# clearmatics/libff

Hardware: AMD Instinct MI355X
Metric: G1 MSM throughput (scalar-muls/sec) (higher is better)
Workload: dtype u32

## Files before the change

libff_amd/csrc/engine.cpp:

```cpp
#include "../../include/amdmsm.h"
#include "engine_internal.h"
#include "group_vtable.h"

#include <hip/hip_runtime.h>

#include <fcntl.h>
#include <sys/stat.h>
#include <unistd.h>

#include <algorithm>
#include <cmath>
#include <cstdio>
#include <cstdlib>
#include <cstring>
#include <mutex>
#include <string>
#include <thread>
#include <vector>

using namespace amdmsm;

constexpr int MAX_SLOTS = 4;
constexpr int MAX_GROUPS = 4;
struct ws_slot {
// ... 207 lines not shown
    while (L < 64u && (size_t)p.W * (size_t)batch * p.B * red_lanes / L > (size_t)70000) L <<= 1;
    if (L_req > 0) L = (uint32_t)L_req;
    while (L > p.B) L >>= 1;
    if (L == 0 || (L & (L - 1))) return AMDMSM_ERR_BAD_ARG;
    p.L = L;
    const size_t xyz_bytes = (size_t)3 * vt->el_words * 4;
    p.list_stride = align_up(n ? n : 1, 64) + 16;
    {
        const double resident = (double)vt->accumulate_resident_lanes(overlap ? 1 : 0);
        const double entries = (double)n * p.W;
        uint32_t S = 8;
        if (entries >= 4.0 * 256.0 * resident) {
            S = 256;
        } else if (entries >= 8.0 * 128.0 * resident) {
            S = 128;
        } else if (entries > 8.0 * resident) {
            uint32_t k = 1;
            while (entries / (k * resident) > 128.0) ++k;
            S = (uint32_t)std::ceil(entries / (k * resident));
            while (S < 128 && (double)p.W * (double)((n + S - 1) / S) > k * resident) ++S;
        }
        if (S_req > 0) S = (uint32_t)S_req;
        p.S = S;
        p.T = (uint32_t)((n + S - 1) / S);
        if (p.T == 0) p.T = 1;
    }
    p.K = batch;
    const size_t Wt = (size_t)p.W * (size_t)batch;
    size_t off = 0;
    p.off_counts = off;
    off = align_up(off + Wt * p.B * 4, 256);
    p.off_lists = off;
    off = align_up(off + Wt * p.list_stride * 4, 256);
    const size_t zz_bytes = (size_t)vt->bucket_words * 4;
    p.off_buckets = off;
    off = align_up(off + Wt * p.B * zz_bytes, 256);
    const size_t M = p.B / p.L;
    p.off_lvl0 = off;
    off = align_up(off + Wt * M * xyz_bytes, 256);
    p.off_lvl1 = off;
    off = align_up(off + Wt * (M / 2 + 1) * xyz_bytes, 256);
    p.off_pfirst = off;
    off = align_up(off + Wt * p.T * zz_bytes, 256);
    p.off_plast = off;
    off = align_up(off + Wt * p.T * zz_bytes, 256);
    p.off_cont = off;
    off = align_up(off + Wt * p.T * 4, 256);
    p.G = G_req > 0 ? std::min(std::min(G_req, MAX_GROUPS), p.W) : 1;
    p.off_queue = off;
    p.queue_stride = align_up(fixup_queue_words((size_t)((p.W + p.G - 1) / p.G) * (size_t)batch * p.T) * 4, 256);
    off = off + p.queue_stride * p.G;
    p.off_partial = off;
    off = align_up(off + (size_t)MAX_GROUPS * xyz_bytes, 256);
    p.off_coarse = off;
    off = align_up(off + Wt * 1025 * 4, 256);
    p.off_big = off;
    p.big_stride = p.c <= 22 ? align_up(sort_geometry(n, p.c, p.W).big_words * 4, 256) : 256;
    off += p.big_stride * (size_t)batch;
    p.off_cursor = off;
    off = align_up(off + Wt * 1024 * 4, 256);
    p.off_tmp_payload = off;
    off = align_up(off + Wt * p.list_stride * 4, 256);
    p.off_tmp_key = off;
    off = align_up(off + Wt * p.list_stride * 4, 256);
    p.off_endo = off;
    p.endo_stride = glv ? align_up((n / 2) * (size_t)vt->el_words * 2 * 4, 256) : 0;
    off += p.endo_stride * (size_t)batch;
    {
        static const int rc_env = getenv("AMDMSM_ROWCOL") ? atoi(getenv("AMDMSM_ROWCOL")) : 1;
        static const int rc_min_c = getenv("AMDMSM_ROWCOL_MIN_C") ? atoi(getenv("AMDMSM_ROWCOL_MIN_C")) : 10;
        static const int qr_env = getenv("AMDMSM_ROWCOL_QROW") ? atoi(getenv("AMDMSM_ROWCOL_QROW")) : 0;
        static const int qc_env = getenv("AMDMSM_ROWCOL_QCOL") ? atoi(getenv("AMDMSM_ROWCOL_QCOL")) : 0;
        p.rowcol = rc_env != 0 && p.c >= rc_min_c;
        const int h = p.c / 2;
        const size_t C = (size_t)1 << h, R = p.B >> h;
        const bool one_wave = vt->fq_words >= 24 || vt->el_words > vt->fq_words;
        const size_t lane_budget = one_wave ? 70000 : 140000;
        uint32_t q = 4;
        while (q < 64 && Wt * p.B * red_lanes * 2 / q > lane_budget) q <<= 1;
        p.q_row = qr_env > 0 ? (uint32_t)qr_env : q;
        p.q_col = qc_env > 0 ? (uint32_t)qc_env : q;
        p.rc_points = R + 1 + C;
        p.off_rc = off;
        off = align_up(off + Wt * p.rc_points * xyz_bytes, 256);
        p.off_planes = off;
        off = align_up(off + Wt * p.c * xyz_bytes, 256);
        p.off_winsum = off;
        off = align_up(off + Wt * xyz_bytes, 256);
    }
    p.total = off;
    return AMDMSM_OK;
}

int ensure_ws(amdmsm_ctx *ctx, ws_slot &sl, size_t bytes) {
    if (sl.ws_bytes >= bytes) return AMDMSM_OK;
    if (sl.ws) {
        HIP_TRY(ctx, hipDeviceSynchronize());
        HIP_TRY(ctx, hipFree(sl.ws));
        sl.ws = nullptr;
        sl.ws_bytes = 0;
    }
    const size_t want = bytes + bytes / 8;
    HIP_TRY(ctx, hipMalloc(&sl.ws, want));
    sl.ws_bytes = want;
    return AMDMSM_OK;
}

constexpr uint64_t TIMING_RING = 64;
void record(amdmsm_ctx *ctx, ws_slot &sl, int idx, hipStream_t st) {
    (void)sl;
    if (ctx->timing) (void)hipEventRecord(ctx->ring[ctx->ticket % TIMING_RING][idx], st);
}

bool use_endomorphism(const group_vtable *vt, size_t n, const amdmsm_opts *opts, int table_digits) {
    static const int env = [] {
        const char *e = getenv("AMDMSM_GLV");
        int v = 0;
        if (!e) return 0;
        if (!strcmp(e, "off") || !strcmp(e, "0")) v = -1;
        else if (!strcmp(e, "on") || !strcmp(e, "1")) v = 1;
        else if (!strcmp(e, "all") || !strcmp(e, "force") || !strcmp(e, "2")) v = 2;
        else if (!strcmp(e, "auto")) v = 3;
        if (v) fprintf(stderr, "[amdmsm] AMDMSM_GLV=%s overrides amdmsm_opts.endomorphism where the caller left it at 0 "
                               "(off: everywhere); on / force assert that every base lies in the order-r subgroup\n", e);
        return v;
    }();
    if (!vt->has_endomorphism) return false;
    if (table_digits || n == 0 || n >= ((size_t)1 << 30)) return false;
    const int c_req = opts ? opts->window_bits : 0;
    if (c_req > 22) return false;
    int want = opts ? opts->endomorphism : 0;
    if (env == -1) want = -1;
    else if ((env == 1 || env == 2) && want == 0) want = env;
    if (want < 0 || (want == 0 && !vt->prime_order)) return false;
    if (want >= 2) return true;
    double full = 0, split = 0;
    if (c_req) {
        full = plan_cost(vt, n, c_req, false);
        split = plan_cost(vt, n, c_req, true);
    } else {
        choose_c(vt, n, false, &full);
        choose_c(vt, n, true, &split);
    }
    return split < 0.98 * full;
}

int check_opts(amdmsm_ctx *ctx, const amdmsm_opts *opts) {
    if (opts && opts->struct_size != sizeof(amdmsm_opts))
        return fail(ctx, AMDMSM_ERR_BAD_ARG, "amdmsm_opts.struct_size does not match this library (AMDMSM_ABI_VERSION " +
                                                 std::to_string(AMDMSM_ABI_VERSION) + "): initialise with AMDMSM_OPTS_INIT");
    return AMDMSM_OK;
}
#define CHECK_OPTS(ctx, opts)                       \
    do {                                            \
        const int rc_opts_ = check_opts(ctx, opts); \
        if (rc_opts_) return rc_opts_;              \
    } while (0)

constexpr size_t MAX_RANGES = 64;
size_t max_range_points() {
    static const size_t v = [] {
        const char *e = getenv("AMDMSM_MAX_RANGE_POINTS");
        const long long x = e ? atoll(e) : 0;
        return x > 0 ? (size_t)x : (size_t)1 << 28;
    }();
    return v;
}
// ... 27 lines not shown
                       groups_env, glv, overlap);
    if (rc) return fail(ctx, rc, "bad window_bits / segment_len");
    const int slot_idx = (int)(ctx->next++ % (unsigned)ctx->depth);
    ws_slot &sl = ctx->slots[slot_idx];
    ctx->last_slot = slot_idx;
    if (overlap) {
        HIP_TRY(ctx, hipEventRecord(sl.ov_in, user_st));
        st = ctx->bulk_stream;
        HIP_TRY(ctx, hipStreamWaitEvent(st, sl.ov_in, 0));
    }
    if (sl.used) HIP_TRY(ctx, hipStreamWaitEvent(st, sl.done, 0));
    rc = ensure_ws(ctx, sl, p.total);
    if (rc) return rc;
    char *ws = (char *)sl.ws;
    uint32_t *counts = (uint32_t *)(ws + p.off_counts);
    uint32_t *lists = (uint32_t *)(ws + p.off_lists);
    uint32_t *buckets = (uint32_t *)(ws + p.off_buckets);
    uint32_t *lvl0 = (uint32_t *)(ws + p.off_lvl0);
    uint32_t *lvl1 = (uint32_t *)(ws + p.off_lvl1);

    record(ctx, sl, 0, st);
    const uint32_t *endo_pts = !glv ? nullptr : (d_endo_resident ? d_endo_resident : (const uint32_t *)(ws + p.off_endo));
    const bool endo_beside = glv && !d_endo_resident && !(hook && hook->fn);
    HIP_TRY(ctx, hipEventRecord(sl.tail_done[0], st));
    if ((atomic_sort || p.c > 22) && !table_digits) {
        HIP_TRY(ctx, hipMemsetAsync(counts, 0, (size_t)p.W * p.B * 4, st));
        vt->count(st, d_scalars, n, mont, p.c, p.W, counts);
        record(ctx, sl, 1, st);
        vt->scatter(st, d_scalars, n, mont, p.c, p.W, counts, lists, p.list_stride);
    } else {
        HIP_TRY(ctx, hipMemsetAsync(ws + p.off_coarse, 0, p.off_big + 16 - p.off_coarse, st));
        record(ctx, sl, 1, st);
        vt->sort(st, d_scalars, n, mont, p.c, table_digits ? table_digits : p.W, (uint32_t *)(ws + p.off_coarse),
                 (uint32_t *)(ws + p.off_cursor), (int32_t *)lists, (uint32_t *)(ws + p.off_tmp_payload),
                 (uint32_t *)(ws + p.off_tmp_key), counts, lists, p.list_stride, (uint32_t *)(ws + p.off_big),
                 table_digits ? 1 : (glv ? 2 : 0), nullptr);
    }
    hipStream_t side = overlap ? st : sl.side[0];
    if (!overlap) HIP_TRY(ctx, hipStreamWaitEvent(side, sl.tail_done[0], 0));
    HIP_TRY(ctx, hipMemsetAsync(buckets, 0, (size_t)p.W * p.B * vt->bucket_words * 4, side));
    for (int g = 0; g < p.G; ++g) HIP_TRY(ctx, hipMemsetAsync(ws + p.off_queue + g * p.queue_stride, 0, 8, side));
    if (endo_beside) vt->endo_points(side, d_bases, n, (uint32_t *)(ws + p.off_endo));
    if (!overlap) HIP_TRY(ctx, hipEventRecord(sl.acc_done[0], side));
    if (hook && hook->fn) {
        hipEvent_t wait_for = nullptr;
        rc = hook->fn(hook->arg, &wait_for);
        if (rc) return rc;
        if (wait_for) HIP_TRY(ctx, hipStreamWaitEvent(st, wait_for, 0));
    }
    if (!overlap) HIP_TRY(ctx, hipStreamWaitEvent(st, sl.acc_done[0], 0));
    if (glv && !d_endo_resident && !endo_beside) vt->endo_points(st, d_bases, n, (uint32_t *)(ws + p.off_endo));
    const size_t zzw = (size_t)vt->bucket_words, xyzw = (size_t)vt->el_words * 3;
    const size_t M0 = p.B / p.L, cap1 = M0 / 2 + 1;
    uint32_t *pfirst = (uint32_t *)(ws + p.off_pfirst), *plast = (uint32_t *)(ws + p.off_plast);
    uint32_t *cont = (uint32_t *)(ws + p.off_cont), *partial = (uint32_t *)(ws + p.off_partial);
    int w_hi = p.W;
    for (int g = 0; g < p.G; ++g) {
        const int wg = p.W / p.G + (g < p.W % p.G ? 1 : 0);
        const int w0 = w_hi - wg;
        w_hi = w0;
        const bool last = g == p.G - 1;
        hipStream_t ts = last ? (overlap ? ctx->tail_stream : st) : sl.side[g];
        if (g == 0) record(ctx, sl, 2, st);
        vt->accumulate(st, counts + (size_t)w0 * p.B, lists + (size_t)w0 * p.list_stride, p.list_stride, d_bases,
                       buckets + (size_t)w0 * p.B * zzw, pfirst + (size_t)w0 * p.T * zzw, plast + (size_t)w0 * p.T * zzw,
                       cont + (size_t)w0 * p.T, wg, p.B, p.S, p.T, endo_pts, n, overlap ? 1 : 0);
        if (last) {
            record(ctx, sl, 3, st);
            if (overlap) {
                HIP_TRY(ctx, hipEventRecord(sl.ov_acc, st));
                HIP_TRY(ctx, hipStreamWaitEvent(ts, sl.ov_acc, 0));
            }
        } else {
            HIP_TRY(ctx, hipEventRecord(sl.acc_done[g], st));
            HIP_TRY(ctx, hipStreamWaitEvent(ts, sl.acc_done[g], 0));
        }
        vt->accumulate_fixup(ts, counts + (size_t)w0 * p.B, buckets + (size_t)w0 * p.B * zzw,
                             pfirst + (size_t)w0 * p.T * zzw, plast + (size_t)w0 * p.T * zzw, cont + (size_t)w0 * p.T,
                             (uint32_t *)(ws + p.off_queue + g * p.queue_stride), wg, p.B, p.S, p.T);
        uint32_t *src = lvl0 + (size_t)w0 * M0 * xyzw, *dst = lvl1 + (size_t)w0 * cap1 * xyzw;
        if (p.rowcol) {
            src = (uint32_t *)(ws + p.off_winsum) + (size_t)w0 * xyzw;
            vt->reduce_rowcol(ts, buckets + (size_t)w0 * p.B * zzw, wg, p.B, p.c, p.q_row, p.q_col,
                              (uint32_t *)(ws + p.off_rc) + (size_t)w0 * p.rc_points * xyzw,
                              (uint32_t *)(ws + p.off_planes) + (size_t)w0 * p.c * xyzw, src);
        } else {
            vt->reduce_segments(ts, buckets + (size_t)w0 * p.B * zzw, wg, p.B, p.L, src);
            const uint32_t fold = (uint32_t)vt->reduce_fold;
            uint32_t M = (uint32_t)M0;
            M /= std::min<uint32_t>(M, fold);
            while (M > 1) {
                if ((size_t)M * (64 / fold) <= 256) {
                    vt->sum_block(ts, src, wg, M, dst);
                    M = 1;
                } else {
                    vt->sum_butterfly(ts, src, wg, M, dst);
                    M /= std::min<uint32_t>(M, fold);
                }
                std::swap(src, dst);
            }
        }
        if (g > 0) HIP_TRY(ctx, hipStreamWaitEvent(ts, sl.tail_done[g - 1], 0));
        if (last) record(ctx, sl, 4, ts);
        vt->horner(ts, src, wg, p.c, last ? form : (int)AMDMSM_OUT_JACOBIAN, g > 0 ? partial + (size_t)(g - 1) * xyzw : nullptr,
                   last ? d_out : partial + (size_t)g * xyzw);
        if (!last) HIP_TRY(ctx, hipEventRecord(sl.tail_done[g], ts));
    }
    if (overlap) {
        record(ctx, sl, 5, ctx->tail_stream);
        HIP_TRY(ctx, hipEventRecord(sl.ov_tail, ctx->tail_stream));
        HIP_TRY(ctx, hipStreamWaitEvent(user_st, sl.ov_tail, 0));
        st = user_st;
    } else {
        record(ctx, sl, 5, st);
    }
    if (ctx->timing) sl.last_ticket = (long long)ctx->ticket++;
    sl.ev_valid = ctx->timing;
    HIP_TRY(ctx, hipEventRecord(sl.done, st));
    sl.used = true;
    HIP_TRY(ctx, hipGetLastError());
    return AMDMSM_OK;
}

constexpr int MAX_BATCH = 8;
int msm_device_batch_impl(amdmsm_ctx *ctx, const group_vtable *vt, int k, const uint32_t *const *d_bases,
                          const uint32_t *const *d_scalars, size_t n, uint32_t *const *d_outs, const amdmsm_opts *opts) {
    hipStream_t st = (opts && opts->stream) ? (hipStream_t)opts->stream : ctx->stream;
    const int form = opts ? opts->out_form : AMDMSM_OUT_LIBFF;
    const int mont = (opts && opts->scalars_plain) ? 0 : 1;
    const bool glv = use_endomorphism(vt, n, opts, 0);
    const size_t entries = glv ? 2 * n : n;
    plan_t p;
    int rc = make_plan(vt, entries, opts ? opts->window_bits : 0, opts ? opts->segment_len : 0, p, 0, 0, 0, glv, false, k);
    if (rc) return fail(ctx, rc, "bad window_bits / segment_len");
    if (p.c > 22) return fail(ctx, AMDMSM_ERR_BAD_ARG, "window_bits > 22 is not available for a batch");
    const int slot_idx = (int)(ctx->next++ % (unsigned)ctx->depth);
    ws_slot &sl = ctx->slots[slot_idx];
    ctx->last_slot = slot_idx;
    if (sl.used) HIP_TRY(ctx, hipStreamWaitEvent(st, sl.done, 0));
    rc = ensure_ws(ctx, sl, p.total);
    if (rc) return rc;
    char *ws = (char *)sl.ws;
    const size_t zzw = (size_t)vt->bucket_words, xyzw = (size_t)vt->el_words * 3;
    const size_t Wt = (size_t)p.W * (size_t)k;
    uint32_t *counts = (uint32_t *)(ws + p.off_counts), *lists = (uint32_t *)(ws + p.off_lists);
    uint32_t *buckets = (uint32_t *)(ws + p.off_buckets);
    uint32_t *pfirst = (uint32_t *)(ws + p.off_pfirst), *plast = (uint32_t *)(ws + p.off_plast), *cont = (uint32_t *)(ws + p.off_cont);
    record(ctx, sl, 0, st);
    HIP_TRY(ctx, hipMemsetAsync(ws + p.off_coarse, 0, Wt * 1025 * 4, st));
    for (int j = 0; j < k; ++j) HIP_TRY(ctx, hipMemsetAsync(ws + p.off_big + (size_t)j * p.big_stride, 0, 16, st));
    HIP_TRY(ctx, hipMemsetAsync(buckets, 0, Wt * p.B * vt->bucket_words * 4, st));
    HIP_TRY(ctx, hipMemsetAsync(ws + p.off_queue, 0, 8, st));
    record(ctx, sl, 1, st);
    for (int j = 0; j < k; ++j) {
        const size_t w0 = (size_t)j * p.W;
        uint32_t *lists_j = lists + w0 * p.list_stride, *counts_j = counts + w0 * p.B;
        vt->sort(st, d_scalars[j], n, mont, p.c, p.W, (uint32_t *)(ws + p.off_coarse) + w0 * 1025,
                 (uint32_t *)(ws + p.off_cursor) + w0 * 1024, (int32_t *)lists_j,
                 (uint32_t *)(ws + p.off_tmp_payload) + w0 * p.list_stride, (uint32_t *)(ws + p.off_tmp_key) + w0 * p.list_stride,
                 counts_j, lists_j, p.list_stride, (uint32_t *)(ws + p.off_big + (size_t)j * p.big_stride), glv ? 2 : 0, nullptr);
        uint32_t *endo_j = glv ? (uint32_t *)(ws + p.off_endo + (size_t)j * p.endo_stride) : nullptr;
        if (glv) vt->endo_points(st, d_bases[j], n, endo_j);
        if (j == 0) record(ctx, sl, 2, st);
        vt->accumulate(st, counts_j, lists_j, p.list_stride, d_bases[j], buckets + w0 * p.B * zzw, pfirst + w0 * p.T * zzw,
                       plast + w0 * p.T * zzw, cont + w0 * p.T, p.W, p.B, p.S, p.T, endo_j, n, 0);
    }
    record(ctx, sl, 3, st);
// ... 1450 lines not shown
```

libff_amd/csrc/msm_group.hip:

```cpp
#include "curve_params.h"
#include "ec.cuh"
#include "fp2h.cuh"
#include "group_vtable.h"
#include "wide.cuh"
#include "wide28.cuh"
#include "rr.cuh"

#include <algorithm>
#include <cstdio>
#include <vector>
#include <type_traits>

#ifndef AMDMSM_GROUP
#error "compile with -DAMDMSM_GROUP=<group traits> -DAMDMSM_VT=<vtable getter name>"
#endif

namespace amdmsm {
template <bool I>
struct ec_coeff_a<Fp<AMDMSM_GROUP::fq, I>> {
    static constexpr int value = AMDMSM_GROUP::DEG == 1 ? AMDMSM_GROUP::COEFF_A : 0;
};
template <int NR, bool I>
struct ec_coeff_a<Fp2<AMDMSM_GROUP::fq, NR, I>> {
    static constexpr int value = AMDMSM_GROUP::DEG == 2 ? AMDMSM_GROUP::COEFF_A : 0;
// ... 1421 lines not shown
    const uint32_t i = (uint32_t)(t % M);
    const bool valid = w < (size_t)W;
    Jac<ER> p;
    if (valid) load_jac(p, in + t * XYZW); else jac_set_inf(p);
    wave_group_sum_r(p, G);
    if (valid && (i % G) == 0) store_jac(out + (w * (M / G) + i / G) * XYZW, p);
}

__global__ void __launch_bounds__(256) k_sum_block(const uint32_t* __restrict__ in, int W, uint32_t M,
                                                    uint32_t* __restrict__ out) {
    __shared__ uint32_t part[4 * XYZW];
    const size_t w = blockIdx.x;
    const uint32_t i = threadIdx.x / RED_LANES;
    const uint32_t lane = threadIdx.x & 63u, wave = threadIdx.x >> 6, nw = blockDim.x >> 6;
    Jac<ER> p;
    if (i < M) load_jac(p, in + (w * M + i) * XYZW); else jac_set_inf(p);
    wave_group_sum_r(p, RED_FOLD);
    if (lane < (uint32_t)RED_LANES) store_jac(part + wave * XYZW, p);
    __syncthreads();
    if (wave != 0) return;
    const uint32_t j = lane / RED_LANES;
    if (j < nw) load_jac(p, part + j * XYZW); else jac_set_inf(p);
    uint32_t G = 1;
    while (G < nw) G <<= 1;
    wave_group_sum_r(p, G);
    if (lane < (uint32_t)RED_LANES) store_jac(out + w * XYZW, p);
}

constexpr int SUMW_THREADS = (GP::DEG == 1 && FQ::N < 16) ? 512 : 256;
constexpr int SUMW_SLOTS = SUMW_THREADS / RED_LANES / 4;
template <class Q = FQ>
AMDMSM_DEV void sum_wide_add(const WideEnv<Q>& env, const uint32_t* a, const uint32_t* b, uint32_t* o) {
    if constexpr (GP::DEG == 2) {
        using F = WideFq2<Q, (GP::NR_SMALL == 0 ? -1 : GP::NR_SMALL)>;
        const uint32_t wi = F::word_index(env);
        uint32_t X1 = env.valid ? a[wi] : 0u, Y1 = env.valid ? a[EW + wi] : 0u, Z1 = env.valid ? a[2 * EW + wi] : 0u;
        const uint32_t X2 = env.valid ? b[wi] : 0u, Y2 = env.valid ? b[EW + wi] : 0u, Z2 = env.valid ? b[2 * EW + wi] : 0u;
        jac_add_seq<F, Q, GP::COEFF_A>(env, X1, Y1, Z1, X2, Y2, Z2);
        if (((threadIdx.x & 63u) >> 4) < 2 && env.valid) {
            o[wi] = X1;
            o[EW + wi] = Y1;
            o[2 * EW + wi] = Z1;
        }
    } else {
        uint32_t X1 = env.valid ? a[env.j] : 0u, Y1 = env.valid ? a[EW + env.j] : 0u, Z1 = env.valid ? a[2 * EW + env.j] : 0u;
        const uint32_t X2 = env.valid ? b[env.j] : 0u, Y2 = env.valid ? b[EW + env.j] : 0u, Z2 = env.valid ? b[2 * EW + env.j] : 0u;
        if constexpr (Q::N < 16) jac_add_wide<Q, GP::COEFF_A>(env, X1, Y1, Z1, X2, Y2, Z2);
        else jac_add_seq<WideFq<Q>, Q>(env, X1, Y1, Z1, X2, Y2, Z2);
        if ((threadIdx.x & 63u) < (uint32_t)Q::N) {
            o[env.j] = X1;
            o[EW + env.j] = Y1;
            o[2 * EW + env.j] = Z1;
        }
    }
}
__global__ void __launch_bounds__(SUMW_THREADS) k_sum_block_wide(const uint32_t* __restrict__ in, int W, uint32_t M,
                                                                 uint32_t* __restrict__ out) {
    __shared__ uint32_t buf[2][SUMW_SLOTS * XYZW];
    __builtin_amdgcn_s_setprio(3);
    const size_t w = blockIdx.x;
    const uint32_t i = threadIdx.x / RED_LANES, wave = threadIdx.x >> 6;
    constexpr uint32_t NWAVES = SUMW_THREADS / 64;
    Jac<ER> p;
    if (i < M) load_jac(p, in + (w * M + i) * XYZW); else jac_set_inf(p);
    wave_group_sum_r(p, 4);
    if ((i & 3u) == 0) store_jac(buf[0] + (size_t)(i >> 2) * XYZW, p);
    __syncthreads();
    const WideEnv<FQ> env = wide_env<FQ>();
    uint32_t K = (M + 3) / 4;
    int cur = 0;
    while (K > 1) {
        const uint32_t pairs = K / 2;
        for (uint32_t q = wave; q < pairs; q += NWAVES) {
            const uint32_t* a = buf[cur] + (size_t)(2 * q) * XYZW;
            sum_wide_add(env, a, a + XYZW, buf[cur ^ 1] + (size_t)q * XYZW);
        }
        __syncthreads();
        cur ^= 1;
        K = pairs;
    }
    for (uint32_t t = threadIdx.x; t < (uint32_t)XYZW; t += SUMW_THREADS) out[w * XYZW + t] = buf[cur][t];
}

__global__ void __launch_bounds__(64, AMDMSM_TAIL_WAVES) k_bucket_sums(const uint32_t* __restrict__ buckets, int W, uint32_t B, int h,
                                                    uint32_t q_row, uint32_t q_col, uint32_t row_blocks,
                                                    uint32_t* __restrict__ out) {
    __builtin_amdgcn_s_setprio(3);
    const bool col = blockIdx.x >= row_blocks;
    const size_t t = ((size_t)(blockIdx.x - (col ? row_blocks : 0u)) * 64 + threadIdx.x) / RED_LANES;
    const uint32_t C = 1u << h, R = B >> h;
    const uint32_t q = col ? q_col : q_row, len = col ? R : C;
    const uint32_t g = len / q;
    const uint32_t nout = col ? C : R + 1;
    const size_t per_w = (size_t)nout * g;
    const size_t w = t / per_w;
    const uint32_t rem = (uint32_t)(t % per_w), o = rem / g, j = rem % g;
    const bool valid = w < (size_t)W;
    rec_sum sum;
    rec_sum_init(sum);
    if (valid) {
        const uint32_t* bk = buckets + w * (size_t)B * ZZS;
        for (uint32_t i = 0; i < q; ++i) {
            const uint32_t idx = j * q + i;
            const uint64_t b1 = col ? (uint64_t)idx * C + o : (uint64_t)o * C + idx;
            if (b1 >= 1 && b1 <= B) rec_sum_add(sum, bk + (size_t)(b1 - 1) * ZZS);
        }
    }
    rec_sum_fold(sum, g);
    Xyzz<ER> xa;
    rec_sum_get(xa, sum);
    Jac<ER> p;
    xyzz_to_jac(p, xa);
    if (valid && j == 0) store_jac(out + (w * (size_t)(R + 1 + C) + (col ? R + 1 + o : o)) * XYZW, p);
}

__global__ void __launch_bounds__(256) k_plane_sums(const uint32_t* __restrict__ rc, int W, int c, int h,
                                                     uint32_t* __restrict__ planes) {
    __shared__ uint32_t part[4 * XYZW];
    __builtin_amdgcn_s_setprio(3);
    const uint32_t w = blockIdx.x / (uint32_t)c, k = blockIdx.x % (uint32_t)c;
    const uint32_t C = 1u << h, R = (1u << (c - 1)) >> h, NP = R + 1 + C;
    const bool from_cols = k < (uint32_t)h;
    const uint32_t* src = rc + ((size_t)w * NP + (from_cols ? R + 1 : 0)) * XYZW;
    const uint32_t bit = from_cols ? k : k - (uint32_t)h;
    const bool top = k == (uint32_t)c - 1;
    const uint32_t M = top ? 1u : (from_cols ? C : R) / 2;
    const uint32_t nlanes = blockDim.x / RED_LANES, i0 = threadIdx.x / RED_LANES;
    const uint32_t lane = threadIdx.x & 63u, wave = threadIdx.x >> 6, nw = blockDim.x >> 6;
    Jac<ER> p, x;
    jac_set_inf(p);
    for (uint32_t i = i0; i < M; i += nlanes) {
        const uint32_t idx = top ? R : (((i >> bit) << (bit + 1)) | (1u << bit) | (i & ((1u << bit) - 1u)));
        load_jac(x, src + (size_t)idx * XYZW);
        jac_add(p, p, x);
    }
    wave_group_sum_r(p, RED_FOLD);
    if (lane < (uint32_t)RED_LANES) store_jac(part + wave * XYZW, p);
    __syncthreads();
    if (wave != 0) return;
    const uint32_t jw = lane / RED_LANES;
    if (jw < nw) load_jac(p, part + jw * XYZW); else jac_set_inf(p);
    uint32_t G = 1;
    while (G < nw) G <<= 1;
    wave_group_sum_r(p, G);
    if (lane < (uint32_t)RED_LANES) store_jac(planes + ((size_t)w * c + k) * XYZW, p);
}

__global__ void __launch_bounds__(SUMW_THREADS) k_plane_sums_wide(const uint32_t* __restrict__ rc, int W, int c, int h,
                                                                  uint32_t* __restrict__ planes) {
    __shared__ uint32_t buf[2][SUMW_SLOTS * XYZW];
    __builtin_amdgcn_s_setprio(3);
    const uint32_t w = blockIdx.x / (uint32_t)c, k = blockIdx.x % (uint32_t)c;
    const uint32_t C = 1u << h, R = (1u << (c - 1)) >> h, NP = R + 1 + C;
    const bool from_cols = k < (uint32_t)h;
    const uint32_t* src = rc + ((size_t)w * NP + (from_cols ? R + 1 : 0)) * XYZW;
    const uint32_t bit = from_cols ? k : k - (uint32_t)h;
    const bool top = k == (uint32_t)c - 1;
    const uint32_t M = top ? 1u : (from_cols ? C : R) / 2;
    constexpr uint32_t NLANES = SUMW_THREADS / RED_LANES, NWAVES = SUMW_THREADS / 64;
    const uint32_t i0 = threadIdx.x / RED_LANES, wave = threadIdx.x >> 6;
    Jac<ER> p, x;
    jac_set_inf(p);
    for (uint32_t i = i0; i < M; i += NLANES) {
        const uint32_t idx = top ? R : (((i >> bit) << (bit + 1)) | (1u << bit) | (i & ((1u << bit) - 1u)));
        load_jac(x, src + (size_t)idx * XYZW);
        jac_add(p, p, x);
    }
    wave_group_sum_r(p, 4);
    if ((i0 & 3u) == 0) store_jac(buf[0] + (size_t)(i0 >> 2) * XYZW, p);
    __syncthreads();
    const WideEnv<FQ> env = wide_env<FQ>();
    uint32_t K = ((M < NLANES ? M : NLANES) + 3) / 4;
    int cur = 0;
    while (K > 1) {
        const uint32_t pairs = K / 2;
        for (uint32_t q = wave; q < pairs; q += NWAVES) {
            const uint32_t* a = buf[cur] + (size_t)(2 * q) * XYZW;
            sum_wide_add(env, a, a + XYZW, buf[cur ^ 1] + (size_t)q * XYZW);
        }
        __syncthreads();
        cur ^= 1;
        K = pairs;
    }
    for (uint32_t t = threadIdx.x; t < (uint32_t)XYZW; t += SUMW_THREADS) planes[((size_t)w * c + k) * XYZW + t] = buf[cur][t];
}

template <class P, bool I>
AMDMSM_DEV typename std::enable_if<(P::N < 16), void>::type horner_chain(Jac<Fp<P, I>>& res,
                                                                         const uint32_t* __restrict__ window_sums, int W,
                                                                         int c, const uint32_t* __restrict__ init) {
    const WideEnv<P> env = wide_env<P>();
    auto load = [&](const uint32_t* p, uint32_t& X, uint32_t& Y, uint32_t& Z) {
        X = env.valid ? p[env.j] : 0u;
        Y = env.valid ? p[EW + env.j] : 0u;
        Z = env.valid ? p[2 * EW + env.j] : 0u;
    };
    uint32_t X, Y, Z, X2, Y2, Z2;
    int w = W - 1;
    if (init) {
        load(init, X, Y, Z);
    } else {
        load(window_sums + (size_t)w * XYZW, X, Y, Z);
        --w;
    }
    for (; w >= 0; --w) {
        if (!wide_is_zero(Z)) {
            if constexpr (GP::COEFF_A != 0) for (int i = 0; i < c; ++i) jac_dbl_wide<P, GP::COEFF_A>(env, X, Y, Z);
            else if (c >= 4) jac_dbl_run28<P>(env, X, Y, Z, c);
            else for (int i = 0; i < c; ++i) jac_dbl_wide<P>(env, X, Y, Z);
        }
        load(window_sums + (size_t)w * XYZW, X2, Y2, Z2);
        jac_add_wide<P, GP::COEFF_A>(env, X, Y, Z, X2, Y2, Z2);
    }
    wide_to_packed(res.x, X);
    wide_to_packed(res.y, Y);
    wide_to_packed(res.z, Z);
}
template <class P, bool I>
AMDMSM_DEV typename std::enable_if<(P::N >= 16 && P::N < 32), void>::type horner_chain(
    Jac<Fp<P, I>>& res, const uint32_t* __restrict__ window_sums, int W, int c, const uint32_t* __restrict__ init) {
    using F = WideFq<P>;
    const WideEnv<P> env = wide_env<P>();
    auto load = [&](const uint32_t* p, uint32_t& X, uint32_t& Y, uint32_t& Z) {
        X = env.valid ? p[env.j] : 0u;
        Y = env.valid ? p[EW + env.j] : 0u;
        Z = env.valid ? p[2 * EW + env.j] : 0u;
    };
    uint32_t X, Y, Z, X2, Y2, Z2;
    int w = W - 1;
    if (init) {
        load(init, X, Y, Z);
    } else {
        load(window_sums + (size_t)w * XYZW, X, Y, Z);
        --w;
    }
    for (; w >= 0; --w) {
        if (!wide_is_zero(Z)) {
            if (c >= 4) jac_dbl_run28<P>(env, X, Y, Z, c);
            else for (int i = 0; i < c; ++i) jac_dbl_wide2<P>(env, X, Y, Z);
        }
        load(window_sums + (size_t)w * XYZW, X2, Y2, Z2);
        jac_add_seq<F, P>(env, X, Y, Z, X2, Y2, Z2);
    }
    wide_to_packed(res.x, X);
    wide_to_packed(res.y, Y);
    wide_to_packed(res.z, Z);
}
template <class P, int NR, bool I>
AMDMSM_DEV typename std::enable_if<(P::N < 16), void>::type horner_chain(Jac<Fp2<P, NR, I>>& res,
                                                                         const uint32_t* __restrict__ window_sums, int W,
                                                                         int c, const uint32_t* __restrict__ init) {
// ... 938 lines not shown
            cap = waves;
        }
        (void)hipMemsetAsync(d_trace, 0, waves * 24, st);
        hipLaunchKernelGGL(k_accumulate, dim3(blocks_for((size_t)W * T * ACC_LANES)), dim3(TPB), dyn_lds, st, ends, lists,
                           list_stride, bases, buckets, part_first, part_last, cont_bucket, W, B, S, T, endo_pts,
                           endo_pts ? (uint32_t)n_real : 0x80000000u, sync_waves, d_trace);
        if (const char* path = getenv("AMDMSM_ACC_TRACE_FILE")) {
            (void)hipStreamSynchronize(st);
            std::vector<unsigned long long> h(waves * 3);
            (void)hipMemcpy(h.data(), d_trace, waves * 24, hipMemcpyDeviceToHost);
            if (FILE* f = fopen(path, "wb")) {
                fwrite(h.data(), 8, h.size(), f);
                fclose(f);
            }
        }
    }
#else
    hipLaunchKernelGGL(k_accumulate, dim3(blocks_for((size_t)W * T * ACC_LANES)), dim3(TPB), dyn_lds, st, ends, lists,
                       list_stride, bases, buckets, part_first, part_last, cont_bucket, W, B, S, T, endo_pts,
                       endo_pts ? (uint32_t)n_real : 0x80000000u, sync_waves);
#endif
}
void l_endo_points(hipStream_t st, const uint32_t* bases, size_t n, uint32_t* out) {
    if (!n) return;
    hipLaunchKernelGGL(k_endo_points, dim3(blocks_for(n * 2 * GP::DEG)), dim3(TPB), 0, st, bases, n, out);
}
void l_glv_digits(hipStream_t st, const uint32_t* scalars, size_t n, int mont, int c, int W, int32_t* out) {
    if (!n) return;
    hipLaunchKernelGGL(k_glv_digits, dim3(blocks_for(n)), dim3(TPB), 0, st, scalars, n, mont, c, W, out);
}
size_t l_accumulate_resident_lanes(int overlap) {
    auto query = [](size_t dyn_lds) {
        int dev = 0, cus = 256, blocks = 0;
        if (hipGetDevice(&dev) == hipSuccess) (void)hipDeviceGetAttribute(&cus, hipDeviceAttributeMultiprocessorCount, dev);
        if (hipOccupancyMaxActiveBlocksPerMultiprocessor(&blocks, k_accumulate, TPB, dyn_lds) != hipSuccess || blocks <= 0) blocks = 4;
        return (size_t)cus * (size_t)blocks * TPB / ACC_LANES;
    };
    static const size_t lanes = query(0);
    static const size_t lanes_overlap = (AMDMSM_OVERLAP_OK && ACC_OVERLAP_LDS) ? query(ACC_OVERLAP_LDS) : lanes;
    return overlap ? lanes_overlap : lanes;
}
void l_accumulate_fixup(hipStream_t st, const uint32_t* ends, uint32_t* buckets, uint32_t* part_first,
                        const uint32_t* part_last, const uint32_t* cont_bucket, uint32_t* queue, int W, uint32_t B,
                        uint32_t S, uint32_t T) {
    const unsigned fix_blocks = blocks_for((size_t)W * T * RED_LANES, 64);
    const unsigned compact_blocks = T / FIX_BLOCK >= 2 ? (unsigned)(W * (T / FIX_BLOCK - 1)) : 0u;
    hipLaunchKernelGGL(k_accumulate_fixup, dim3(fix_blocks + compact_blocks), dim3(64), 0, st, ends, part_first,
                       part_last, cont_bucket, buckets, queue, W, B, S, T, fix_blocks);
    const size_t lanes = (size_t)W * T;
    const size_t cap_mid = fixup_queue_cap_mid(lanes) / (RED_FOLD / MID_G) + 1, cap_long = fixup_queue_cap_long(lanes);
    const unsigned mid_blocks = (unsigned)(cap_mid < 8192 ? cap_mid : 8192), long_blocks = (unsigned)(cap_long < 2048 ? cap_long : 2048);
    hipLaunchKernelGGL(k_accumulate_fixup_queue, dim3(mid_blocks + long_blocks), dim3(64), 0, st, ends,
                       part_first, part_last, cont_bucket, buckets, queue, mid_blocks, lanes, B, S, T);
}
void l_reduce_segments(hipStream_t st, const uint32_t* buckets, int W, uint32_t B, uint32_t L, uint32_t* out) {
    hipLaunchKernelGGL(k_reduce_segments, dim3(blocks_for((size_t)W * (B / L) * RED_LANES, 64)), dim3(64), 0, st, buckets, W, B,
                       L, out);
}
void l_sum_butterfly(hipStream_t st, const uint32_t* in, int W, uint32_t M, uint32_t* out) {
    hipLaunchKernelGGL(k_sum_butterfly, dim3(blocks_for((size_t)W * M * RED_LANES, 64)), dim3(64), 0, st, in, W, M, out);
}
void l_sum_block(hipStream_t st, const uint32_t* in, int W, uint32_t M, uint32_t* out) {
    if (M >= 8 && M * RED_LANES <= (uint32_t)SUMW_THREADS && (M & (M - 1)) == 0) {
        hipLaunchKernelGGL(k_sum_block_wide, dim3(W), dim3(SUMW_THREADS), 0, st, in, W, M, out);
        return;
    }
    const unsigned threads = (unsigned)((M * RED_LANES + 63) / 64 * 64);
    hipLaunchKernelGGL(k_sum_block, dim3(W), dim3(threads), 0, st, in, W, M, out);
}
void l_reduce_rowcol(hipStream_t st, const uint32_t* buckets, int W, uint32_t B, int c, uint32_t q_row, uint32_t q_col,
                     uint32_t* rc, uint32_t* planes, uint32_t* out) {
    const int h = c / 2;
    const uint32_t C = 1u << h, R = B >> h;
    auto fit = [](uint32_t len, uint32_t q) {
        if (q < 1) q = 1;
        while (q & (q - 1)) q &= q - 1;
        if (q > len) q = len;
        while (len / q > RED_FOLD) q <<= 1;
        return q;
    };
    q_row = fit(C, q_row);
    q_col = fit(R, q_col);
    const size_t row_lanes = (size_t)W * (R + 1) * (C / q_row) * RED_LANES, col_lanes = (size_t)W * C * (R / q_col) * RED_LANES;
    const unsigned row_blocks = blocks_for(row_lanes, 64), col_blocks = blocks_for(col_lanes, 64);
    hipLaunchKernelGGL(k_bucket_sums, dim3(row_blocks + col_blocks), dim3(64), 0, st, buckets, W, B, h, q_row, q_col, row_blocks, rc);
    const uint32_t maxm = (C > R ? C : R) / 2;
    static const bool wide_planes = !(getenv("AMDMSM_PLANES_WIDE") && atoi(getenv("AMDMSM_PLANES_WIDE")) == 0);
    if (maxm >= 8 && wide_planes) {
        hipLaunchKernelGGL(k_plane_sums_wide, dim3((unsigned)(W * c)), dim3(SUMW_THREADS), 0, st, rc, W, c, h, planes);
    } else {
        unsigned threads = (unsigned)((maxm * RED_LANES + 63) / 64 * 64);
        threads = threads < 64 ? 64 : (threads > 256 ? 256 : threads);
        hipLaunchKernelGGL(k_plane_sums, dim3((unsigned)(W * c)), dim3(threads), 0, st, rc, W, c, h, planes);
    }
    hipLaunchKernelGGL(k_window_horner, dim3((unsigned)W), dim3((unsigned)(64 * ((c + 3) / 4))), 0, st, planes, c, out);
}
void l_horner(hipStream_t st, const uint32_t* window_sums, int W, int c, int form, const uint32_t* init, uint32_t* out) {
    hipLaunchKernelGGL(k_horner, dim3(1), dim3(64), 0, st, window_sums, W, c, form, init, out);
}
void l_horner_batch(hipStream_t st, const uint32_t* window_sums, int k, int W, int c, int form, uint32_t* const* outs) {
    horner_outs o = {};
    for (int j = 0; j < k && j < 8; ++j) o.p[j] = outs[j];
    hipLaunchKernelGGL(k_horner_batch, dim3((unsigned)k), dim3(64), 0, st, window_sums, W, c, form, o);
}
void l_sum_points(hipStream_t st, const uint32_t* pts, int k, int form, uint32_t* out) {
    hipLaunchKernelGGL(k_sum_points, dim3(1), dim3(64), 0, st, pts, k, form, out);
}
void l_gen_bases_seq(hipStream_t st, unsigned long long first, size_t n, uint32_t* dst) {
    if (!n) return;
    hipLaunchKernelGGL(k_gen_bases_seq, dim3(blocks_for(n)), dim3(TPB), 0, st, first, n, dst);
}
void l_export_affine(hipStream_t st, const uint32_t* src, size_t n, uint32_t* dst) {
    if (!n) return;
    hipLaunchKernelGGL(k_export_affine, dim3(blocks_for(n)), dim3(TPB), 0, st, src, n, dst);
}
void l_ffi_decode_points(hipStream_t st, const uint32_t* src, size_t n, uint32_t* dst, uint32_t* status) {
    if (!n) return;
    hipLaunchKernelGGL(k_ffi_decode_points, dim3(blocks_for(n)), dim3(TPB), 0, st, src, n, dst, status);
}
void l_ffi_decode_scalars(hipStream_t st, const uint32_t* src, size_t n, uint32_t* dst, uint32_t* status) {
    if (!n) return;
    hipLaunchKernelGGL(k_ffi_decode_scalars, dim3(blocks_for(n)), dim3(TPB), 0, st, src, n, dst, status);
}
void l_ffi_encode_point(hipStream_t st, const uint32_t* src_xyz, uint32_t* dst) {
    hipLaunchKernelGGL(k_ffi_encode_point, dim3(1), dim3(64), 0, st, src_xyz, dst);
}
void l_disk_decode(hipStream_t st, const uint32_t* src, size_t n, uint32_t* dst) {
    if (!n) return;
    hipLaunchKernelGGL(k_disk_decode, dim3(blocks_for(n)), dim3(TPB), 0, st, src, n, dst);
}
void l_disk_decode_compressed(hipStream_t st, const uint32_t* src, size_t n, uint32_t* dst, uint32_t* status) {
    if (!n) return;
    hipLaunchKernelGGL(k_disk_decode_compressed, dim3(blocks_for(n, 64)), dim3(64), 0, st, src, n, dst, status);
}
#if AMDMSM_ACC_RR
template <class G>
bool launch_fb_exp_rr(hipStream_t st, const uint32_t* table_aff, const uint32_t* scalars, size_t n, int mont, const uint32_t* coeff,
                      int scalar_size, int window, int form, uint32_t* out) {
    if constexpr (G::DEG == 1) {
        if (window < 32) {
            hipLaunchKernelGGL(k_fb_exp_rr<G>, dim3(blocks_for(n)), dim3(TPB), 0, st, table_aff, scalars, n, mont, coeff, scalar_size,
                               window, form, out);
            return true;
        }
    }
    return false;
}
#endif
void l_fixed_base_exp(hipStream_t st, const uint32_t* g_xyz, int scalar_size, int window, const uint32_t* scalars, size_t n,
                      int mont, const uint32_t* coeff, int form, uint32_t* gouter, uint32_t* table, uint32_t* table_aff,
                      int build_table, uint32_t* out) {
    const int outerc = (scalar_size + window - 1) / window;
    if (build_table) {
        hipLaunchKernelGGL(k_fb_gouter, dim3(1), dim3(64), 0, st, g_xyz, outerc, window, gouter);
        for (int level = 0; level < window; ++level) {
            const size_t per_level = level == 0 ? 2 : ((size_t)1 << level);
            hipLaunchKernelGGL(k_fb_table_level, dim3(blocks_for((size_t)outerc * per_level)), dim3(TPB), 0, st, gouter, outerc,
                               window, scalar_size, level, table);
        }
        const size_t entries = (size_t)outerc << window;
        hipLaunchKernelGGL(k_fb_table_affine, dim3(blocks_for((entries + FB_NORM_K - 1) / FB_NORM_K)), dim3(TPB), 0, st, table,
                           entries, table_aff);
    }
    if (n) {
#if AMDMSM_ACC_RR
        if (launch_fb_exp_rr<GP>(st, table_aff, scalars, n, mont, coeff, scalar_size, window, form, out)) return;
#endif
        hipLaunchKernelGGL(k_fb_exp, dim3(blocks_for(n)), dim3(TPB), 0, st, table_aff, scalars, n, mont, coeff, scalar_size,
// ... 54 lines not shown
```

Measured before the change: 617.2 million.

## Keep row/column sums in XYZZ form and fold partials through LDS

The row/column bucket-sum kernel now runs with larger workgroups and merges its partial sums through shared memory instead of the wave-level fold. It writes the results in XYZZ bucket format rather than converting them to Jacobian. The plane-sum kernels then accumulate these XYZZ points with the cheaper rec_sum add path and convert to Jacobian only once at the end. The aim is to cut the per-point Jacobian conversions and the costly jac_add work in the reduction tail, at the cost of LDS traffic, extra barriers and possibly lower occupancy.

```diff
diff --git a/libff_amd/csrc/engine.cpp b/libff_amd/csrc/engine.cpp
--- a/libff_amd/csrc/engine.cpp
+++ b/libff_amd/csrc/engine.cpp
@@ -313,7 +313,7 @@
         p.q_col = qc_env > 0 ? (uint32_t)qc_env : q;
         p.rc_points = R + 1 + C;
         p.off_rc = off;
-        off = align_up(off + Wt * p.rc_points * xyz_bytes, 256);
+        off = align_up(off + Wt * p.rc_points * (size_t)vt->bucket_words * 4, 256);
         p.off_planes = off;
         off = align_up(off + Wt * p.c * xyz_bytes, 256);
         p.off_winsum = off;
@@ -507,7 +507,7 @@
         if (p.rowcol) {
             src = (uint32_t *)(ws + p.off_winsum) + (size_t)w0 * xyzw;
             vt->reduce_rowcol(ts, buckets + (size_t)w0 * p.B * zzw, wg, p.B, p.c, p.q_row, p.q_col,
-                              (uint32_t *)(ws + p.off_rc) + (size_t)w0 * p.rc_points * xyzw,
+                              (uint32_t *)(ws + p.off_rc) + (size_t)w0 * p.rc_points * zzw,
                               (uint32_t *)(ws + p.off_planes) + (size_t)w0 * p.c * xyzw, src);
         } else {
             vt->reduce_segments(ts, buckets + (size_t)w0 * p.B * zzw, wg, p.B, p.L, src);
diff --git a/libff_amd/csrc/msm_group.hip b/libff_amd/csrc/msm_group.hip
--- a/libff_amd/csrc/msm_group.hip
+++ b/libff_amd/csrc/msm_group.hip
@@ -1527,36 +1527,76 @@
     for (uint32_t t = threadIdx.x; t < (uint32_t)XYZW; t += SUMW_THREADS) out[w * XYZW + t] = buf[cur][t];
 }
 
-__global__ void __launch_bounds__(64, AMDMSM_TAIL_WAVES) k_bucket_sums(const uint32_t* __restrict__ buckets, int W, uint32_t B, int h,
+constexpr int RS_WORDS = (int)((sizeof(rec_sum) + 3) / 4);
+constexpr int BS_THREADS = RS_WORDS * 4 * 256 <= 64 * 1024 ? 256 : 128;
+constexpr uint32_t BS_LANES = BS_THREADS / RED_LANES;
+static_assert(BS_LANES >= RED_FOLD, "a row or column sum lies within one workgroup");
+AMDMSM_DEV void rec_sum_to_lds(uint32_t* lds, uint32_t slot, const rec_sum& s) {
+    uint32_t w[RS_WORDS] = {};
+    __builtin_memcpy(w, &s, sizeof(rec_sum));
+#pragma unroll
+    for (int k = 0; k < RS_WORDS; ++k) lds[k * BS_THREADS + slot] = w[k];
+}
+AMDMSM_DEV void rec_sum_from_lds(rec_sum& s, const uint32_t* lds, uint32_t slot) {
+    uint32_t w[RS_WORDS];
+#pragma unroll
+    for (int k = 0; k < RS_WORDS; ++k) w[k] = lds[k * BS_THREADS + slot];
+    __builtin_memcpy(&s, w, sizeof(rec_sum));
+}
+AMDMSM_DEV void rec_sum_merge(rec_sum& s, const rec_sum& o) {
+#if AMDMSM_SUM_RR
+    xyzz_add_rho(s.a, s.inf, o.a, o.inf);
+#else
+    xyzz_add(s.a, s.a, o.a);
+#endif
+}
+__global__ void __launch_bounds__(BS_THREADS, AMDMSM_TAIL_WAVES) k_bucket_sums(const uint32_t* __restrict__ buckets, int W, uint32_t B, int h,
                                                     uint32_t q_row, uint32_t q_col, uint32_t row_blocks,
                                                     uint32_t* __restrict__ out) {
+    __shared__ uint32_t part[RS_WORDS * BS_THREADS];
     __builtin_amdgcn_s_setprio(3);
     const bool col = blockIdx.x >= row_blocks;
-    const size_t t = ((size_t)(blockIdx.x - (col ? row_blocks : 0u)) * 64 + threadIdx.x) / RED_LANES;
+    const uint32_t rl = threadIdx.x / RED_LANES, sub = threadIdx.x % RED_LANES;
+    const size_t t0 = (size_t)(blockIdx.x - (col ? row_blocks : 0u)) * BS_LANES;
     const uint32_t C = 1u << h, R = B >> h;
     const uint32_t q = col ? q_col : q_row, len = col ? R : C;
     const uint32_t g = len / q;
     const uint32_t nout = col ? C : R + 1;
     const size_t per_w = (size_t)nout * g;
-    const size_t w = t / per_w;
-    const uint32_t rem = (uint32_t)(t % per_w), o = rem / g, j = rem % g;
-    const bool valid = w < (size_t)W;
     rec_sum sum;
     rec_sum_init(sum);
-    if (valid) {
-        const uint32_t* bk = buckets + w * (size_t)B * ZZS;
-        for (uint32_t i = 0; i < q; ++i) {
-            const uint32_t idx = j * q + i;
-            const uint64_t b1 = col ? (uint64_t)idx * C + o : (uint64_t)o * C + idx;
-            if (b1 >= 1 && b1 <= B) rec_sum_add(sum, bk + (size_t)(b1 - 1) * ZZS);
-        }
-    }
-    rec_sum_fold(sum, g);
-    Xyzz<ER> xa;
-    rec_sum_get(xa, sum);
-    Jac<ER> p;
-    xyzz_to_jac(p, xa);
-    if (valid && j == 0) store_jac(out + (w * (size_t)(R + 1 + C) + (col ? R + 1 + o : o)) * XYZW, p);
+    {
+        const size_t t = t0 + rl, w = t / per_w;
+        const uint32_t rem = (uint32_t)(t % per_w), o = rem / g, j = rem % g;
+        if (w < (size_t)W) {
+            const uint32_t* bk = buckets + w * (size_t)B * ZZS;
+            for (uint32_t i = 0; i < q; ++i) {
+                const uint32_t idx = j * q + i;
+                const uint64_t b1 = col ? (uint64_t)idx * C + o : (uint64_t)o * C + idx;
+                if (b1 >= 1 && b1 <= B) rec_sum_add(sum, bk + (size_t)(b1 - 1) * ZZS);
+            }
+        }
+    }
+    const uint32_t ns = BS_LANES / g;
+    if (g > 1) {
+        rec_sum_to_lds(part, threadIdx.x, sum);
+        __syncthreads();
+    }
+    for (uint32_t m = g; m > 1; m >>= 1) {
+        const uint32_t half = m >> 1;
+        if (rl < ns * half) {
+            const uint32_t base = rl / half * g + rl % half;
+            rec_sum o;
+            rec_sum_from_lds(sum, part, base * RED_LANES + sub);
+            rec_sum_from_lds(o, part, (base + half) * RED_LANES + sub);
+            rec_sum_merge(sum, o);
+            if (half > 1) rec_sum_to_lds(part, base * RED_LANES + sub, sum);
+        }
+        if (half > 1) __syncthreads();
+    }
+    const size_t sg = t0 / g + rl, w = sg / nout;
+    const uint32_t o = (uint32_t)(sg % nout);
+    if (rl < ns && w < (size_t)W) rec_sum_store(out + (w * (size_t)(R + 1 + C) + (col ? R + 1 + o : o)) * ZZS, sum);
 }
 
 __global__ void __launch_bounds__(256) k_plane_sums(const uint32_t* __restrict__ rc, int W, int c, int h,
@@ -1566,20 +1606,23 @@
     const uint32_t w = blockIdx.x / (uint32_t)c, k = blockIdx.x % (uint32_t)c;
     const uint32_t C = 1u << h, R = (1u << (c - 1)) >> h, NP = R + 1 + C;
     const bool from_cols = k < (uint32_t)h;
-    const uint32_t* src = rc + ((size_t)w * NP + (from_cols ? R + 1 : 0)) * XYZW;
+    const uint32_t* src = rc + ((size_t)w * NP + (from_cols ? R + 1 : 0)) * ZZS;
     const uint32_t bit = from_cols ? k : k - (uint32_t)h;
     const bool top = k == (uint32_t)c - 1;
     const uint32_t M = top ? 1u : (from_cols ? C : R) / 2;
     const uint32_t nlanes = blockDim.x / RED_LANES, i0 = threadIdx.x / RED_LANES;
     const uint32_t lane = threadIdx.x & 63u, wave = threadIdx.x >> 6, nw = blockDim.x >> 6;
-    Jac<ER> p, x;
-    jac_set_inf(p);
+    rec_sum sum;
+    rec_sum_init(sum);
     for (uint32_t i = i0; i < M; i += nlanes) {
         const uint32_t idx = top ? R : (((i >> bit) << (bit + 1)) | (1u << bit) | (i & ((1u << bit) - 1u)));
-        load_jac(x, src + (size_t)idx * XYZW);
-        jac_add(p, p, x);
-    }
-    wave_group_sum_r(p, RED_FOLD);
+        rec_sum_add(sum, src + (size_t)idx * ZZS);
+    }
+    rec_sum_fold(sum, RED_FOLD);
+    Xyzz<ER> xa;
+    rec_sum_get(xa, sum);
+    Jac<ER> p;
+    xyzz_to_jac(p, xa);
     if (lane < (uint32_t)RED_LANES) store_jac(part + wave * XYZW, p);
     __syncthreads();
     if (wave != 0) return;
@@ -1598,20 +1641,23 @@
     const uint32_t w = blockIdx.x / (uint32_t)c, k = blockIdx.x % (uint32_t)c;
     const uint32_t C = 1u << h, R = (1u << (c - 1)) >> h, NP = R + 1 + C;
     const bool from_cols = k < (uint32_t)h;
-    const uint32_t* src = rc + ((size_t)w * NP + (from_cols ? R + 1 : 0)) * XYZW;
+    const uint32_t* src = rc + ((size_t)w * NP + (from_cols ? R + 1 : 0)) * ZZS;
     const uint32_t bit = from_cols ? k : k - (uint32_t)h;
     const bool top = k == (uint32_t)c - 1;
     const uint32_t M = top ? 1u : (from_cols ? C : R) / 2;
     constexpr uint32_t NLANES = SUMW_THREADS / RED_LANES, NWAVES = SUMW_THREADS / 64;
     const uint32_t i0 = threadIdx.x / RED_LANES, wave = threadIdx.x >> 6;
-    Jac<ER> p, x;
-    jac_set_inf(p);
+    rec_sum sum;
+    rec_sum_init(sum);
     for (uint32_t i = i0; i < M; i += NLANES) {
         const uint32_t idx = top ? R : (((i >> bit) << (bit + 1)) | (1u << bit) | (i & ((1u << bit) - 1u)));
-        load_jac(x, src + (size_t)idx * XYZW);
-        jac_add(p, p, x);
-    }
-    wave_group_sum_r(p, 4);
+        rec_sum_add(sum, src + (size_t)idx * ZZS);
+    }
+    rec_sum_fold(sum, 4);
+    Xyzz<ER> xa;
+    rec_sum_get(xa, sum);
+    Jac<ER> p;
+    xyzz_to_jac(p, xa);
     if ((i0 & 3u) == 0) store_jac(buf[0] + (size_t)(i0 >> 2) * XYZW, p);
     __syncthreads();
     const WideEnv<FQ> env = wide_env<FQ>();
@@ -2716,8 +2762,8 @@
     q_row = fit(C, q_row);
     q_col = fit(R, q_col);
     const size_t row_lanes = (size_t)W * (R + 1) * (C / q_row) * RED_LANES, col_lanes = (size_t)W * C * (R / q_col) * RED_LANES;
-    const unsigned row_blocks = blocks_for(row_lanes, 64), col_blocks = blocks_for(col_lanes, 64);
-    hipLaunchKernelGGL(k_bucket_sums, dim3(row_blocks + col_blocks), dim3(64), 0, st, buckets, W, B, h, q_row, q_col, row_blocks, rc);
+    const unsigned row_blocks = blocks_for(row_lanes, BS_THREADS), col_blocks = blocks_for(col_lanes, BS_THREADS);
+    hipLaunchKernelGGL(k_bucket_sums, dim3(row_blocks + col_blocks), dim3(BS_THREADS), 0, st, buckets, W, B, h, q_row, q_col, row_blocks, rc);
     const uint32_t maxm = (C > R ? C : R) / 2;
     static const bool wide_planes = !(getenv("AMDMSM_PLANES_WIDE") && atoi(getenv("AMDMSM_PLANES_WIDE")) == 0);
     if (maxm >= 8 && wide_planes) {
```

New measurement: 622.4 million (median of 6 runs). Within noise of the previous version (+0.8%).
